# iagostorch/VVC-Affine-GPU

Hardware: AMD Instinct MI355X
Metric: candidate CU-blocks/s at 1080p QP32; bit-exact CPMV/cost match vs reference (higher is better)
Workload: dtype int32; 1 GPU; 1920x1080 QP32, 2 frames, 2-CPMV affine only (FULL+HALF CUs); resolution=1920x1080, qp=32, sequence_frames=2, sequence_pairs=3, pocs_rank0=2, modes=2cp, parallelism=frame-shard x1 (a sequence of its own per rank)

## Files before the change

### profiles/count_preds.py

```python
#!/usr/bin/env python3
import argparse
import ctypes
import json
import os
import sys

R = os.path.dirname(os.path.dirname(os.path.abspath(__file__)))
sys.path.insert(0, os.path.join(R, "vvc-affine-gpu_amd"))
sys.path.insert(0, R)

import torch

from bench import CONFIGS
from vame import _lib
from vame.engine import Engine
from vame.metrics import pair_accounting
from vame.seqrun import ShardRun


def main():
    ap = argparse.ArgumentParser()
    ap.add_argument("--config", default="c2", choices=sorted(CONFIGS))
    ap.add_argument("--qp", type=int, default=None)
    ap.add_argument("--gpus", type=int, default=1)
    ap.add_argument("--rank-only", type=int, default=0, help="count rank K's block of a --gpus N job")
    args = ap.parse_args()
    cfg = CONFIGS[args.config]
    qp = cfg["qp"] if args.qp is None else args.qp
    L = _lib.lib()
    if not hasattr(L, "vame_debug_pred_count"):
        raise SystemExit("VAME_LIB must point at the instrumentation build (make count)")
    L.vame_debug_pred_count.argtypes = [ctypes.c_void_p, ctypes.c_int]
    torch.cuda.set_device(0)
    dev = torch.device("cuda", 0)
    eng = Engine(cfg["W"], cfg["H"], 0)
    n_pairs = None
    if cfg["scaling"] == "weak":
        from vame.shard import frames_for_pairs, sequence_pairs
        n_pairs = sequence_pairs(cfg["frames"]) * args.gpus
    frames = cfg["frames"] if n_pairs is None else frames_for_pairs(n_pairs)
    run = ShardRun(eng, cfg["W"], cfg["H"], qp, frames, cfg["modes"], args.gpus, args.rank_only, dev,
                   n_pairs=n_pairs)
    cnt = (ctypes.c_ulonglong * 20)()
    L.vame_debug_pred_count(cnt, 1)
    run.step()
    torch.cuda.synchronize()
    L.vame_debug_pred_count(cnt, 1)
    acc = pair_accounting(cfg["W"], cfg["H"], (2, 3) if cfg["modes"] & 2 else (2,))
    alg_q, alg_b = acc["sb_pred_quad"] * run.pairs, acc["sb_pred_big"] * run.pairs
    out = {"config": args.config, "qp": qp, "pairs": run.pairs, "rank": [args.rank_only, args.gpus],
           "executed_quad": cnt[0], "algorithmic_quad": alg_q, "executed_pred_frac_quad": cnt[0] / alg_q,
           "executed_ctu": cnt[1], "algorithmic_ctu": alg_b, "executed_pred_frac_ctu": cnt[1] / alg_b,
           "executed_pred_frac": (cnt[0] + cnt[1]) / (alg_q + alg_b),
           "outside_tile_frac_quad": (cnt[2] + cnt[3]) / max(cnt[0], 1),
           "outside_tile_frac_ctu": (cnt[4] + cnt[5]) / max(cnt[1], 1),
           "outside_tile_quad_2cp_3cp": [cnt[2], cnt[3]], "outside_tile_ctu_2cp_3cp": [cnt[4], cnt[5]],
           "outside_held_by_wider_margin_quad": [cnt[6], cnt[7], cnt[8]],
           "outside_held_by_wider_margin_ctu": [cnt[9], cnt[10], cnt[11]],
           "lane_use_quad": cnt[0] / max(cnt[12], 1), "lane_use_ctu": cnt[1] / max(cnt[13], 1),
           "multi_cu_wave_slots_frac_quad": cnt[14] / max(cnt[12], 1),
           "multi_cu_wave_lane_use_quad": cnt[16] / max(cnt[14], 1)}
    print(json.dumps(out))
    eng.close()


if __name__ == "__main__":
    main()
```

### vvc-affine-gpu_amd/csrc/vame_engine.hip

```cpp
#include <hip/hip_ext.h>
#include <hip/hip_runtime.h>

#include <algorithm>
#include <cstdio>
#include <cstdlib>
#include <cstring>
#include <vector>

#include "../../include/vame.h"
#include "vame_kernel.h"
#include "vame_mc_core.h"
#include "vame_partition.h"
#include "vame_bipred.h"
#include "vame_ctx.h"
#include "vame_templates.h"

#if VAME_SPLIT_TU
namespace vame {
VAME_2CP_KERNELS(extern)
}
#endif

using namespace vame;

// ... 403 lines not shown
      pa.ref = jb.refs[r];
      pa.lambda = jb.lambda;
      for (int m = 0; m < 4; m++) {
        pa.cost[m] = jb.out->cost[r][m];
        pa.cpmv[m] = reinterpret_cast<vame_cpmvs_dev*>(jb.out->cpmvs[r][m]);
      }
      const bool last = j == njobs - 1 && r == jb.nrefs - 1;
      if (kp.nPairs == c->maxPairs || last) {
        kps.push_back(kp);
        kp.nPairs = 0;
      }
    }
  }
  return launch(c, kps, doFull, doHalf, doFull, (hipStream_t)stream);
}

int vame_affine_me_poc(vame_ctx* c, const uint16_t* cur, const uint16_t* const* refs, int nrefs,
                       float lambda, int mode_mask, int extra, const vame_poc_result* out,
                       void* stream) {
  if (!out) return VAME_E_INVALID;
  const vame_poc_job job{cur, refs, nrefs, lambda, out};
  return vame_affine_me_batch(c, &job, 1, mode_mask, extra, stream);
}

int vame_set_prof(vame_ctx* c, int enable) {
  if (!c) return VAME_E_INVALID;
  c->prof = enable != 0;
  return VAME_OK;
}

int vame_set_timing(vame_ctx* c, int enable) {
  if (!c) return VAME_E_INVALID;
  const bool keep = (enable & VAME_TIMING_KEEP) != 0;
  enable &= ~VAME_TIMING_KEEP;
  c->timing = enable == 2 ? (1 | 64) : enable != 0 ? (1 << kTimingClasses) - 1 : 0;
  if (!keep)
    for (size_t& u : c->evUsed) u = 0;
  return VAME_OK;
}

int vame_get_timing(vame_ctx* c, int cls, double* total_ms, int* launches, int reset) {
  if (!c || cls < 0 || cls >= kTimingClasses || !total_ms || !launches) return VAME_E_INVALID;
  DeviceGuard guard(c->device);
  VAME_HIP(guard.err);
  double t = 0;
  for (size_t i = 0; i < c->evUsed[cls]; i++) {
    float ms = 0;
    VAME_HIP(hipEventSynchronize(c->ev[cls][i].second));
    VAME_HIP(hipEventElapsedTime(&ms, c->ev[cls][i].first, c->ev[cls][i].second));
    t += ms;
  }
  *total_ms = t;
  *launches = (int)c->evUsed[cls];
  if (reset) c->evUsed[cls] = 0;
  return VAME_OK;
}

const char* vame_strerror(int code) {
  switch (code) {
    case VAME_OK: return "ok";
    case VAME_E_INVALID: return "invalid argument";
    case VAME_E_DEVICE: return "HIP runtime error";
    case VAME_E_NOMEM: return "out of memory";
    case VAME_E_UNSUPPORTED: return "unsupported";
    default: return "unknown error";
  }
}

const char* vame_last_hip_error(void) { return g_hip_err; }

#if VAME_PHASE_TIMING
int vame_debug_phase_cycles(unsigned long long* out, int reset) {
  if (!out) return VAME_E_INVALID;
  VAME_HIP(hipDeviceSynchronize());
  VAME_HIP(hipMemcpyFromSymbol(out, HIP_SYMBOL(g_phase_cycles), sizeof(g_phase_cycles)));
  if (reset) {
    unsigned long long z[7 * kPhSlots] = {};
    VAME_HIP(hipMemcpyToSymbol(HIP_SYMBOL(g_phase_cycles), z, sizeof(z)));
  }
  return VAME_OK;
}
#endif
#if VAME_COUNT_PRED
int vame_debug_pred_count(unsigned long long* out20, int reset) {
  if (!out20) return VAME_E_INVALID;
  VAME_HIP(hipDeviceSynchronize());
  VAME_HIP(hipMemcpyFromSymbol(out20, HIP_SYMBOL(g_pred_count), sizeof(unsigned long long) * 20));
  if (reset) {
    unsigned long long z[20] = {};
    VAME_HIP(hipMemcpyToSymbol(HIP_SYMBOL(g_pred_count), z, sizeof(z)));
  }
  return VAME_OK;
}
#endif
const char* vame_version(void) { return "vame 0.1 (gfx950)"; }

}
```

### vvc-affine-gpu_amd/csrc/vame_instr.h

```cpp
#pragma once
#include <hip/hip_runtime.h>

namespace vame {

#ifndef VAME_ABLATE
#define VAME_ABLATE 0
#endif
#ifndef VAME_DUP
#define VAME_DUP 0
#endif

#ifndef VAME_COUNT_PRED
#define VAME_COUNT_PRED 0
#endif
#if VAME_COUNT_PRED
__device__ unsigned long long g_pred_count[20];
#define PC_DECL unsigned pc_n = 0, pc_w = 0, pc_mw = 0, pc_me = 0;
#define PC_ADD                                                           \
  {                                                                      \
    pc_n++;                                                              \
    const unsigned long long m_ = __builtin_amdgcn_ballot_w64(true);     \
    if (__lane_id() == __builtin_ctzll(m_)) {                            \
      pc_w += 64;                                                        \
      if (!coop && logS < 6) {                                           \
        pc_mw += 64;                                                     \
        pc_me += __popcll(m_);                                           \
      }                                                                  \
    }                                                                    \
  }
#define PC_FLUSH                                                                                \
  {                                                                                             \
    if (pc_n) atomicAdd(&g_pred_count[REGION == 128], (unsigned long long)pc_n);               \
    if (pc_w) atomicAdd(&g_pred_count[12 + (REGION == 128)], (unsigned long long)pc_w);        \
    if (pc_mw) atomicAdd(&g_pred_count[14 + (REGION == 128)], (unsigned long long)pc_mw);      \
    if (pc_me) atomicAdd(&g_pred_count[16 + (REGION == 128)], (unsigned long long)pc_me);      \
  }
#else
#define PC_DECL
#define PC_ADD
#define PC_FLUSH
#endif

#ifndef VAME_PHASE_TIMING
#define VAME_PHASE_TIMING 0
#endif
enum { kPhStage, kPhPredict, kPhCost, kPhGradient, kPhSolve, kPhTail, kPhReduce, kNumPhases };
#if VAME_PHASE_TIMING
constexpr int kPhSlots = 2 * kNumPhases + 4;
__device__ unsigned long long g_phase_cycles[7][kPhSlots];
#define PH_DECL unsigned long long ph_acc[2 * kNumPhases] = {}; unsigned long long ph_t = __builtin_amdgcn_s_memtime(); const unsigned long long ph_t0 = ph_t;
#define PH_MARK(i) { const unsigned long long t_ = __builtin_amdgcn_s_memtime(); ph_acc[(i) + ph_off] += t_ - ph_t; ph_t = t_; }
__shared__ unsigned long long s_ph_blk[3];
__shared__ int s_ph_done;
#define PH_FLUSH { \
  if (lane == 0) { \
    for (int i_ = 0; i_ < 2 * kNumPhases; i_++) atomicAdd(&g_phase_cycles[KIND][i_], ph_acc[i_]); \
    const unsigned long long t1_ = __builtin_amdgcn_s_memtime(); \
    atomicMax(&s_ph_blk[1], t1_); \
    atomicAdd(&s_ph_blk[2], t1_ - ph_t0); \
    const int nw_ = (int)(blockDim.x >> 6); \
    if (atomicAdd(&s_ph_done, 1) == nw_ - 1) { \
      atomicAdd(&g_phase_cycles[KIND][2 * kNumPhases], (unsigned long long)nw_ * (s_ph_blk[1] - s_ph_blk[0])); \
      atomicAdd(&g_phase_cycles[KIND][2 * kNumPhases + 1], s_ph_blk[2]); \
      atomicAdd(&g_phase_cycles[KIND][2 * kNumPhases + 2], 1ull); \
      atomicAdd(&g_phase_cycles[KIND][2 * kNumPhases + 3], s_ph_blk[1] - s_ph_blk[0]); \
    } \
  } }
#define PH_INIT { if (tid == 0) { s_ph_blk[0] = ~0ull; s_ph_blk[1] = 0; s_ph_blk[2] = 0; s_ph_done = 0; } }
#define PH_START { if (lane == 0) atomicMin(&s_ph_blk[0], ph_t0); }
#elif defined(VAME_ISA_MARKS)
#define PH_DECL
#define PH_MARK(i) asm volatile("; PHASE_END " #i);
#define PH_FLUSH
#define PH_INIT
#define PH_START
#else
#define PH_DECL
#define PH_MARK(i)
#define PH_FLUSH
#define PH_INIT
#define PH_START
#endif

}
```

### vvc-affine-gpu_amd/csrc/vame_items.h

```cpp
#pragma once
#include <stdint.h>

namespace vame {

constexpr int kMaxCu = 16;
constexpr int kMaxTasks = 16;
constexpr int kTaskCu = 4;
constexpr int kItemCu = kMaxTasks * kTaskCu;
constexpr int kThreads = 256;

struct CuSlot {
  uint8_t x, y;
  uint8_t lw : 4, lh : 4;
  uint8_t align : 1;
  uint8_t taskCus : 5;
  uint16_t outOff : 9;
  uint16_t taskLogL : 4;
  uint16_t pad;
};
static_assert(sizeof(CuSlot) == 8, "CuSlot packing");

struct Item {
  int16_t nCu;
  int16_t rx, ry;
  int16_t coop;
  int16_t nTasks;
  int16_t rw, rh;
  int16_t pad;
  CuSlot cu[kItemCu];
};

enum { kKindQuad = 0, kKindCtu = 1, kKindHalf = 2, kKindCtu2 = 3, kKindHalf2W = 4, kKindHalf2H = 5, kKindQuad2 = 6 };
template <int KIND>
struct Cfg {
  static constexpr bool HALF2 = KIND == kKindHalf2W || KIND == kKindHalf2H;
  static constexpr bool QUAD = KIND == kKindQuad || KIND == kKindQuad2;
  static constexpr int REGION = QUAD ? 64 : 128;
  static constexpr int THREADS = QUAD || HALF2 ? 256 : KIND == kKindCtu ? 1024 : 512;
  static constexpr int SBL = KIND == kKindCtu2 || HALF2 || KIND == kKindQuad2 ? 2 : 1;
  static constexpr int MAXCU = (KIND == kKindHalf || KIND == kKindCtu2 || HALF2) ? 1 : kMaxCu;
  static constexpr int ITEMCU = QUAD ? kItemCu : MAXCU;
  static constexpr bool AUTO = QUAD;
  static constexpr bool COOP = KIND != kKindQuad2;
  static constexpr int MARGIN = 16;
  static constexpr int TILE = REGION + 2 * MARGIN;
  static constexpr int TILE_W = KIND == kKindHalf2H ? 64 + 2 * MARGIN : TILE;
  static constexpr int TILE_H = KIND == kKindHalf2W ? 64 + 2 * MARGIN : TILE;
  static constexpr int TP = (TILE_W + 7) / 16 * 16 + 8;
  static constexpr int TILE_ELEMS = TILE_H * TP + 16;
  static constexpr int NSB = THREADS * SBL;
  static constexpr bool STASH = KIND != kKindQuad2 && !HALF2;
};

struct BiCand {
  int32_t xy;
  int32_t shape;
  int32_t row;
  int32_t first;
};

}
```

### vvc-affine-gpu_amd/csrc/vame_kernel.h

```cpp
#pragma once
#include <hip/hip_runtime.h>

#include "vame_dev.h"
#include "vame_items.h"

namespace vame {

struct PairArgs {
  const uint16_t* cur;
  const uint16_t* ref;
  int64_t* cost[4];
  vame_cpmvs_dev* cpmv[4];
  float lambda;
  int32_t pad;
};
constexpr int kMaxPairs = 32;

struct KParams {
  PairArgs pair[kMaxPairs];
  const vame_cpmvs_dev* prev[2];
  int32_t* bestS;
  const Item* items;
  const int32_t* order;
  int nItems, nCtus, nPairs;
  int groupPairs, groupPer;
  int nChunks, cpp;
  int W, H, ctusPerRow;
  int extra;
  int run2, run3;
};

constexpr int kSolvePrio = 3;

struct CuState {
  int32_t cur[6];
  int32_t prev[6];
  int32_t best[6];
  int64_t bestCost;
  int64_t bestCostSnap;
  int32_t satd;
  int32_t inframe;
  int32_t live;
  int32_t rate;
  int32_t bestSatd;
  int32_t bestHasS;
  int32_t seedSkip;
  int32_t pad;
};

template <int LOGS>
__device__ __forceinline__ int seg_sum_c(int v) {
  if (LOGS > 0) v += dpp32<0x111, 0xF>(v);
  if (LOGS > 1) v += dpp32<0x112, 0xF>(v);
  if (LOGS > 2) v += dpp32<0x114, 0xF>(v);
  if (LOGS > 3) v += dpp32<0x118, 0xF>(v);
  if (LOGS > 4) v += dpp32<0x142, 0xA>(v);
  if (LOGS > 5) v += dpp32<0x143, 0xC>(v);
  return v;
}


constexpr unsigned long long kLaneBitMask[2] = {0xAAAAAAAAAAAAAAAAull, 0xCCCCCCCCCCCCCCCCull};
template <int B>
__device__ __forceinline__ int sel_bit(int if0, int if1) {
  int r;
  asm("v_cndmask_b32_e64 %0, %1, %2, %3" : "=v"(r) : "v"(if0), "v"(if1), "s"(kLaneBitMask[B]));
  return r;
}
template <int B>
__device__ __forceinline__ long long sel_bit64(long long if0, long long if1) {
  const int lo = sel_bit<B>((int)(unsigned long long)if0, (int)(unsigned long long)if1);
  const int hi = sel_bit<B>((int)((unsigned long long)if0 >> 32), (int)((unsigned long long)if1 >> 32));
  return (long long)(((unsigned long long)(unsigned)hi << 32) | (unsigned)lo);
}
template <int B>
__device__ __forceinline__ long long partner64(long long v) {
  static_assert(B == 0 || B == 1, "quad bits only");
  constexpr int ctrl = B == 1 ? 0x4E : 0xB1;
  const int lo = (int)(unsigned long long)v, hi = (int)((unsigned long long)v >> 32);
  const int rl = dpp32<ctrl, 0xF>(lo), rh = dpp32<ctrl, 0xF>(hi);
  return (long long)(((unsigned long long)(unsigned)rh << 32) | (unsigned)rl);
}
template <int B>
__device__ __forceinline__ long long xchg_masked64(long long a, long long b) {
  unsigned al = (unsigned)(unsigned long long)a, ah = (unsigned)((unsigned long long)a >> 32);
  const unsigned bl = (unsigned)(unsigned long long)b, bh = (unsigned)((unsigned long long)b >> 32);
  if constexpr (B == 3) {
// ... 257 lines not shown
  const int CPR = w.tileW / 8;
  const int NCH = w.tileH * CPR;
  if (w.regionOut) return;
#pragma unroll
  for (int j = 0; j < kStagePer<KIND>; j++) {
    const int ch = tid + j * C::THREADS;
    if (ch < NCH) *reinterpret_cast<uint4*>(&s_tile[(ch / CPR) * C::TP + (ch % CPR) * 8]) = tv[j];
  }
}

template <int KIND>
__device__ __forceinline__ void publish_item(const Item* it, int tid, CuSlot* s_cu, uint4* s_coef,
                                             uint8_t* s_eqmap, int* s_hdr, long long* s_val) {
  using C = Cfg<KIND>;
  if (tid < C::ITEMCU) s_cu[tid] = it->cu[tid];
  if (tid < 48) s_coef[tid] = reinterpret_cast<const uint4*>(&kCoefTab)[tid];
  if (tid < 76) s_eqmap[tid] = kEqMap.v[tid];
  if (tid == 0) {
    s_hdr[0] = it->coop | (it->nTasks << 16);
    s_hdr[1] = 4;
  }
  for (int i = tid; i < C::MAXCU * kNumMom; i += C::THREADS) s_val[i] = 0;
}

struct TaskCtx {
  int tid, lane, wv;
  int cuB, cuE;
  int logL;
  int logS;
  int nCuW;
  int myCu;
  int local;
  int sbIdx;
  int sx, sy;
  int sbCols;
  bool active;
  bool leader;
  Geo g;
};
template <int KIND>
__device__ __forceinline__ TaskCtx task_lanes(const ItemCtx& w, int tid, bool coop, const CuSlot* s_cu) {
  constexpr int SBL = Cfg<KIND>::SBL;
  TaskCtx t;
  t.tid = tid;
  t.lane = tid & 63;
  t.wv = tid >> 6;
  const int lidx = coop ? tid : t.lane;
  const CuSlot t0 = s_cu[coop ? 0 : t.wv * kTaskCu];
  int cuB = coop ? 0 : t.wv * kTaskCu;
  int cuE = cuB + t0.taskCus;
  int logL = t0.taskLogL;
  t.cuB = __builtin_amdgcn_readfirstlane(cuB);
  t.cuE = __builtin_amdgcn_readfirstlane(cuE);
  t.logL = __builtin_amdgcn_readfirstlane(logL);
  t.logS = min(t.logL, 6);
  t.nCuW = coop ? (t.wv == 0 ? t.cuE : 0) : t.cuE - t.cuB;
  const int kLane = t.cuB + (lidx >> t.logL);
  t.myCu = kLane < t.cuE ? kLane : -1;
  t.g.x = t.g.y = t.g.lw = t.g.lh = t.g.w = t.g.h = 0;
  t.local = lidx & ((1 << t.logL) - 1);
  t.sbIdx = 0;
  t.sx = 0;
  t.sy = 0;
  t.sbCols = 1;
  t.active = false;
  if (t.myCu >= 0) {
    const CuSlot cs = s_cu[t.myCu];
    t.g.lw = cs.lw;
    t.g.lh = cs.lh;
    t.g.w = 1 << t.g.lw;
    t.g.h = 1 << t.g.lh;
    t.g.x = w.ctuX + cs.x;
    t.g.y = w.ctuY + cs.y;
    t.sbIdx = tid;
    t.sbCols = 1 << (t.g.lw - 2);
    t.sx = (t.local & (t.sbCols - 1)) << 2;
    t.sy = (t.local >> (t.g.lw - 2)) << (SBL == 2 ? 3 : 2);
    t.active = (t.g.x + t.g.w <= w.W) && (t.g.y + t.g.h <= w.H);
  }
  t.leader = t.myCu >= 0 && (t.lane & ((1 << t.logS) - 1)) == (1 << t.logS) - 1;
  return t;
}

template <int KIND>
__device__ __forceinline__ void take_task_slots(int next, int li, int dstBase, CuSlot* s_cu) {
  if (li < kTaskCu) s_cu[dstBase + li] = s_cu[min(next, Cfg<KIND>::ITEMCU / kTaskCu - 1) * kTaskCu + li];
}

__device__ __forceinline__ int seg_sum(int logS, int v) {
  return logS == 4 ? seg_sum_c<4>(v) : logS == 5 ? seg_sum_c<5>(v) : seg_sum_c<6>(v);
}
__device__ __forceinline__ uint4 ext_row_dpp(const uint2& p) {
  return ext_row(p, dpp32<0x138, 0xF>((int)p.y), dpp32<0x130, 0xF>((int)p.x));
}
__device__ __forceinline__ int bcast_lane7(int v) { return __builtin_amdgcn_update_dpp(0, v, 0x157, 0xF, 0xF, false); }

template <int SBL>
__device__ __forceinline__ void publish_rows(const uint2 (&Pr)[SBL][4], int idx, uint2* s_top, uint2* s_bot,
                                             uint4 (&X)[6]) {
  if constexpr (SBL == 1) {
#pragma unroll
    for (int r = 0; r < 4; r++) X[r + 1] = ext_row_dpp(Pr[0][r]);
  }
  s_top[idx] = Pr[0][0];
  s_bot[idx] = Pr[SBL - 1][3];
}

template <int THREADS>
__device__ __forceinline__ void edge_rows(int idx, int sbCols, const uint2* s_top, const uint2* s_bot, uint2& tb,
                                          uint2& bt) {
  tb = s_bot[max(idx - sbCols, 0)];
  bt = s_top[min(idx + sbCols, THREADS - 1)];
}

template <int ncp, bool STORE>
__device__ __forceinline__ int update_lanes(int loc, const double* M, CuState& st, int cx, int cy, int W, int H) {
  int f = 0, q = 0;
  if (loc < 2 * ncp) {
    const int j = loc;
    const double d = M[j == 1 ? 2 : j == 2 ? 1 : j];
    const int cj = st.cur[j], pj = st.prev[j];
    const int v = update_cpmv(cj, d, (j & 1) ? cy : cx, (j & 1) ? H : W);
    f = (v != cj ? 1 : 0) | (v != pj ? 16 : 0);
    if constexpr (STORE) {
      st.prev[j] = cj;
      st.cur[j] = v;
    }
    q = to_quarter(v);
  }
  const int q2 = dpp32<0x112, 0xF>(q), q4 = dpp32<0x114, 0xF>(q);
  if (loc < 2 * ncp) f += eg_bits(q - (loc >= 4 ? q4 : loc >= 2 ? q2 : 0)) << 8;
  f += dpp32<0x111, 0xF>(f);
  f += dpp32<0x112, 0xF>(f);
  f += dpp32<0x114, 0xF>(f);
  return f;
}

template <int ncp, bool coop, bool keepS, int kDup>
__device__ __forceinline__ bool solve_update_phase(const ItemCtx& w, const TaskCtx& t, const CuSlot* s_cu,
                                                   CuState* s_st, long long (*s_val)[kNumMom], double (*s_mat)[42],
                                                   const uint8_t* s_eqmap) {
  int cuS = t.myCu, loc = t.local;
  opaque(cuS);
  opaque(loc);
  const bool solver = cuS >= 0 && loc < 64;
  const bool act = solver && s_st[cuS].live;
  const int Ls = 1 << t.logS;
  double dd[6] = {0, 0, 0, 0, 0, 0};
  long long* V = s_val[cuS < 0 ? 0 : cuS];
  double* M = s_mat[cuS < 0 ? 0 : cuS];
  const CuSlot cs = s_cu[cuS < 0 ? 0 : cuS];
  if constexpr ((kDup & 16) != 0) {
    double dd2[6] = {0, 0, 0, 0, 0, 0};
    double* M2 = M;
    seg_solve<ncp, true>(V, M2, s_eqmap, loc, Ls, act, coop, cs.lw, cs.lh, dd2);
    asm volatile("" ::"v"(dd2[0]), "v"(dd2[1]), "v"(dd2[3]));
    wave_sync();
  }
  seg_solve<ncp>(V, M, s_eqmap, loc, Ls, act, coop, cs.lw, cs.lh, dd);
  if (keepS && coop && solver && loc == 7) {
    CuState& st = s_st[cuS];
    st.bestCostSnap = st.bestCost;
    st.satd = 0;
  }
  const int cx = w.ctuX + cs.x, cy = w.ctuY + cs.y;
  if constexpr ((kDup & 2048) != 0) {
// ... 34 lines not shown
  const CuSlot cs = s_cu[k];
  const int mode = cs.align * 2 + (ncp - 2);
  const size_t idx = (size_t)w.ctu * (cs.align ? kHalfCusPerCtu : kFullCusPerCtu) + cs.outOff;
  pa.cost[mode][idx] = st.bestCost;
  vame_cpmvs_dev o;
  o.ncps = ncp;
  o.ltx = st.best[0]; o.lty = st.best[1]; o.rtx = st.best[2];
  o.rty = st.best[3]; o.lbx = st.best[4]; o.lby = st.best[5];
  pa.cpmv[mode][idx] = o;
}

template <int KIND, bool PROF, int MODE, typename L>
__device__ __forceinline__ void affine_me_body(const KParams& p, L& lds) {
  constexpr bool run2 = (MODE & 1) != 0, run3 = (MODE & 2) != 0;
  using C = Cfg<KIND>;
  constexpr int REGION = C::REGION;
  (void)REGION;
  static_assert((C::TP * 2) % 16 == 0 && C::TILE_W % 8 == 0, "16-byte tile rows");
  constexpr int SBL = C::SBL;
  constexpr bool STASH = SBL == 2 && C::STASH;
  using Own = Lds<KIND, run2 && run3>;
  static_assert(sizeof(L::tile) >= sizeof(Own::tile) && sizeof(L::top) >= sizeof(Own::top) &&
                    sizeof(L::bestS) >= sizeof(Own::bestS) && sizeof(L::pred) >= sizeof(Own::pred) &&
                    sizeof(L::val) >= sizeof(Own::val) && sizeof(L::mat) >= sizeof(Own::mat) &&
                    sizeof(L::st) >= sizeof(Own::st) && sizeof(L::cu) >= sizeof(Own::cu),
                "LDS layout too small for this kernel class");
  uint16_t* s_tile = lds.tile;
  uint2* s_top = lds.top;
  uint2* s_bot = lds.bot;
  auto& s_bestS = lds.bestS;
  auto& s_pred = lds.pred;
  auto& s_val = lds.val;
  auto& s_mat = lds.mat;
  uint4* s_coef = lds.coef;
  uint8_t* s_eqmap = lds.eqmap;
  CuState* s_st = lds.st;
  CuSlot* s_cu = lds.cu;
  int* s_hdr = lds.hdr;
  __shared__ long long s_dup[(VAME_DUP & 4) ? kNumMom : 1];

  const int tid = threadIdx.x;
  [[maybe_unused]] const int lane = tid & 63;
  const int wv = tid >> 6;
  constexpr int ph_off = 0;
  (void)ph_off;
  PH_DECL
  PC_DECL

  ItemCtx w;
  if (!locate_item<KIND>(p, w)) return;
  const PairArgs& pa = p.pair[w.pairIdx];
  const uint16_t* __restrict__ ref = w.ref;
  const uint16_t* __restrict__ cur = w.cur;
  const int W = w.W, H = w.H, ctu = w.ctu, ctuX = w.ctuX, ctuY = w.ctuY, pairIdx = w.pairIdx, itemIdx = w.itemIdx;
  const int tx0 = w.tx0, ty0 = w.ty0, tileW = w.tileW, tileH = w.tileH;
  uint4 tv[kStagePer<KIND>];
  if constexpr ((VAME_DUP & 64) != 0) {
    int tid2 = tid;
    opaque(tid2);
    stage_load<KIND>(w, tid2, tv);
    stage_store<KIND>(w, tid2, tv, s_tile);
    __syncthreads();
  }
  stage_load<KIND>(w, tid, tv);
  publish_item<KIND>(w.it, tid, s_cu, s_coef, s_eqmap, s_hdr, &s_val[0][0]);
  PH_INIT
  stage_store<KIND>(w, tid, tv, s_tile);
  __syncthreads();
  PH_START
  const int hdr = __builtin_amdgcn_readfirstlane(s_hdr[0]);
  const int nTasks = (hdr >> 16) & 0xFF;
  const bool coop = C::COOP && (!C::AUTO || (hdr & 1) != 0);
  const bool claim = C::AUTO && (hdr & 2) != 0;
  PH_MARK(kPhStage)
  if (!coop && wv >= nTasks) {
    PH_FLUSH
    return;
  }

  const int tidItem = tid;
  for (int task = coop ? 0 : __builtin_amdgcn_readfirstlane(wv);;) {
    int tidTask = tidItem;
    opaque(tidTask);
    const TaskCtx t = task_lanes<KIND>(w, tidTask, coop, s_cu);
    const int tid = t.tid, lane = t.lane, wv = t.wv, cuB = t.cuB, logS = t.logS, nCuW = t.nCuW;
    const int myCu = t.myCu, local = t.local, sbIdx = t.sbIdx, sx = t.sx, sy = t.sy, sbCols = t.sbCols;
    const bool active = t.active, leader = t.leader;
    const Geo g = t.g;
    auto run_pass = [&](auto ncpTag, auto coopTag, auto keepTag) {
      constexpr int ncp = decltype(ncpTag)::value;
      constexpr bool coop = decltype(coopTag)::value;
      constexpr bool keepS = decltype(keepTag)::value;
      constexpr int ph_off = ncp == 3 ? kNumPhases : 0;
      (void)ph_off;
      constexpr int kDup = (VAME_DUP & 32) && ncp != 3 ? 0 : VAME_DUP;
      const int niter = (ncp == 3 ? 4 : 5) + p.extra;

      if (lane < nCuW) {
        int k = __lane_id();
        opaque(k);
        k += cuB;
        const CuSlot cs = s_cu[k];
        CuState& st = s_st[k];
        const int cx = ctuX + cs.x, cy = ctuY + cs.y;
        int c[6] = {0, 0, 0, 0, 0, 0};
        if (ncp == 3) {
          int prev[4];
          if (run2) {
            for (int i = 0; i < 4; i++) prev[i] = st.best[i];
          } else {
            const vame_cpmvs_dev& pv =
                p.prev[cs.align][(size_t)ctu * (cs.align ? kHalfCusPerCtu : kFullCusPerCtu) + cs.outOff];
            prev[0] = pv.ltx; prev[1] = pv.lty; prev[2] = pv.rtx; prev[3] = pv.rty;
          }
          int lbx, lby;
          derive_lb(prev[0], prev[1], prev[2], prev[3], cs.lw, cs.lh, cx, cy, W, H, lbx, lby);
          c[0] = prev[0]; c[1] = prev[1]; c[2] = prev[2]; c[3] = prev[3]; c[4] = lbx; c[5] = lby;
          int skip = 0, satd0 = 0;
          if (run2 && st.bestHasS) {
            const int hx = shl(prev[2] - prev[0], 7 - cs.lw), hy = shl(prev[3] - prev[1], 7 - cs.lw);
            const int vx = shl(lbx - prev[0], 7 - cs.lh), vy = shl(lby - prev[1], 7 - cs.lh);
            if (vx == -hy && vy == hx) {
              skip = 1;
              satd0 = st.bestSatd;
            }
          }
          st.seedSkip = skip;
          st.satd = satd0;
        } else {
          st.satd = 0;
          st.bestHasS = 0;
        }
        int never = (int)0x80000000;
        int costInit = (int)kCostInit;
        opaque(never);
        opaque(costInit);
        for (int i = 0; i < 6; i++) {
          st.cur[i] = c[i];
          st.prev[i] = never;
          st.best[i] = c[i];
        }
        st.bestCost = (long long)costInit;
        st.bestCostSnap = (long long)costInit;
        st.rate = affine_bits(c, ncp);
        st.inframe = (cx + (1 << cs.lw) <= W) && (cy + (1 << cs.lh) <= H);
        st.live = st.inframe;
      }
      phase_sync(coop);

      for (int iter = 0; iter <= niter; iter++) {
        uint2 Pr[SBL][4], Og[SBL][4];
        uint4 X[6];
        const bool live = active && s_st[myCu < 0 ? 0 : myCu].live;
        const bool reuse = ncp == 3 && iter == 0 && s_st[myCu < 0 ? 0 : myCu].seedSkip;
        if (live && !reuse && !(VAME_ABLATE & 8)) {
          PC_ADD
          Geo gp = g;
          int sxp = sx, syp = sy;
          opaque_geo(gp, sxp, syp);
          int cp[6];
          for (int i = 0; i < 6; i++) cp[i] = s_st[myCu].cur[i];
          const MvField f = mv_field(cp, ncp, gp.lw, gp.lh);
          if constexpr ((kDup & 128) != 0) {
            int cp2[6];
            for (int i = 0; i < 6; i++) cp2[i] = cp[i];
            int lw2 = gp.lw;
            opaque(cp2[0]);
            opaque(lw2);
            const MvField f2 = mv_field(cp2, ncp, lw2, gp.lh);
            if (ncp == 3)
              asm volatile("" ::"v"(f2.bx), "v"(f2.by), "v"(f2.hx), "v"(f2.hy), "v"(f2.vx), "v"(f2.vy),
                           "v"((int)f2.spread));
            else
              asm volatile("" ::"v"(f2.bx), "v"(f2.by), "v"(f2.hx), "v"(f2.hy), "v"((int)f2.spread));
          }
          int satdLane = 0;
#pragma unroll
          for (int j = 0; j < SBL; j++) {
            bool outside;
            satdLane += predict_sb<C::TILE, C::TP, PROF, (VAME_ABLATE & 1024) != 0 && ncp == 3, ncp>(
                f, sxp, syp + 4 * j, gp, s_tile, tx0, ty0, tileW - 9, tileH - 9, ref, cur, W, H, s_coef, Pr[j],
                Og[j], outside);
            if (SBL == 2 && j == 0) {
#pragma unroll
              for (int r = 0; r < 4; r++)
                if constexpr (STASH) s_pred[r][sbIdx] = Pr[0][r];
            }
#if VAME_COUNT_PRED
            {
              const unsigned long long out = __builtin_amdgcn_ballot_w64(outside);
              if (out && __lane_id() == __builtin_ctzll(__builtin_amdgcn_ballot_w64(true)))
                atomicAdd(&g_pred_count[2 + 2 * (REGION == 128) + (ncp == 3)], (unsigned long long)__popcll(out));
            }
            if (j > 0) PC_ADD
#endif
          }
          if (kDup & 1) {
            MvField f2 = f;
            opaque(f2.bx);
            uint2 P2[4], O2[4];
            bool out2;
            int s2 = predict_sb<C::TILE, C::TP, PROF>(f2, sxp, syp, gp, s_tile, tx0, ty0, tileW - 9, tileH - 9,
                                                      ref, cur, W, H, s_coef, P2, O2, out2);
            s2 += (int)(P2[0].x ^ P2[3].y ^ O2[1].x);
            asm volatile("" ::"v"(s2));
          }
          publish_rows<SBL>(Pr, sbIdx, s_top, s_bot, X);
          if constexpr ((kDup & 256) != 0) {
            int i2 = sbIdx;
            opaque(i2);
            uint2 Q[SBL][4];
#pragma unroll
            for (int j = 0; j < SBL; j++)
#pragma unroll
              for (int r = 0; r < 4; r++) {
                Q[j][r] = Pr[j][r];
                opaque(reinterpret_cast<int&>(Q[j][r].x));
              }
            uint4 X2[6];
            publish_rows<SBL>(Q, i2, s_top, s_bot, X2);
            if constexpr (SBL == 1) {
#pragma unroll
              for (int r = 0; r < 4; r++) asm volatile("" ::"v"(X2[r + 1].x), "v"(X2[r + 1].w));
            }
          }
          if constexpr ((kDup & 512) != 0) {
            int s2 = satdLane;
            opaque(s2);
            const int v2 = seg_sum(logS, s2);
            asm volatile("" ::"v"(v2));
          }
          const int v = seg_sum(logS, satdLane);
          if (leader) {
            if (coop)
              atomicAdd(&s_st[myCu].satd, v);
            else
              s_st[myCu].satd = v;
          }
        }
        phase_sync(coop);
        PH_MARK(kPhPredict)

        const bool lastIter = iter == niter;
        bool better = false;
        if constexpr ((kDup & 1024) != 0) {
          int bet2 = 0;
          if (myCu >= 0 && (keepS || local == 7)) {
            const CuState& st = s_st[myCu];
            int r2 = st.rate;
            opaque(r2);
            if (iter == 0 || st.live) bet2 = price(st.satd, pa.lambda, r2) < st.bestCost;
          }
          if (!keepS) bet2 = bcast_lane7(bet2);
          asm volatile("" ::"v"(bet2));
        }
        if constexpr (!keepS) {
          int bet = 0;
          if (myCu >= 0 && local == 7) {
            CuState& st = s_st[myCu];
            if (iter == 0 || st.live) {
              const long long cost = price(st.satd, pa.lambda, st.rate);
              if (cost < st.bestCost) {
                st.bestCost = cost;
                bet = 1;
              }
            }
            st.satd = 0;
          }
          bet = bcast_lane7(bet);
          if (myCu >= 0 && local < 6 && bet) s_st[myCu].best[local] = s_st[myCu].cur[local];
        } else {
          if (myCu >= 0) {
            CuState& st = s_st[myCu];
            if (iter == 0 || st.live) {
              const long long cost = price(st.satd, pa.lambda, st.rate);
              better = cost < (coop ? st.bestCostSnap : st.bestCost);
              if (better && local == 7) {
                st.bestCost = cost;
                st.bestSatd = st.satd;
                st.bestHasS = !lastIter && st.live;
              }
            }
            if (local < 6 && better) st.best[local] = st.cur[local];
          }
        }
        PH_MARK(kPhCost)
        if (lastIter) {
          phase_sync(coop);
          break;
        }

        {
          int S[SBL][5];
#pragma unroll
          for (int j = 0; j < SBL; j++)
#pragma unroll
            for (int k = 0; k < 5; k++) S[j][k] = 0;
          char* gBest = SBL == 2 ? reinterpret_cast<char*>(p.bestS + ((size_t)(pairIdx * p.nCtus + ctu) * p.nItems +
                                                                      itemIdx) * 5 * C::NSB)
                                 : nullptr;
          auto gbest = [&](int k, int j) -> int32_t& {
            int i = sbIdx;
            opaque(i);
            return *reinterpret_cast<int32_t*>(gBest + (unsigned)(k * C::NSB + j * C::THREADS + i) * 4u);
          };
          if (reuse && live) {
#pragma unroll
            for (int j = 0; j < SBL; j++)
#pragma unroll
              for (int k = 0; k < 5; k++) S[j][k] = SBL == 1 ? s_bestS[k][sbIdx] : gbest(k, j);
          } else if (live && !(VAME_ABLATE & 2)) {
            int nbIdx = sbIdx;
            if constexpr (SBL == 2) opaque(nbIdx);
            uint2 tb, bt;
            edge_rows<C::THREADS>(nbIdx, sbCols, s_top, s_bot, tb, bt);
            X[0] = ext_row_dpp(tb);
            if constexpr ((kDup & 256) != 0) {
              int n2 = nbIdx;
              opaque(n2);
              uint2 tb2, bt2;
              edge_rows<C::THREADS>(n2, sbCols, s_top, s_bot, tb2, bt2);
              const uint4 a2 = ext_row_dpp(tb2), b2 = ext_row_dpp(bt2);
              asm volatile("" ::"v"(a2.x), "v"(a2.w), "v"(b2.x), "v"(b2.w));
            }
            Geo gg = g;
            int sxg = sx, syg = sy;
            if constexpr (SBL == 2) opaque_geo(gg, sxg, syg);
            if constexpr (SBL == 1) {
              X[5] = ext_row_dpp(bt);
              grad_sb(sxg, syg, gg, X, Og[0], S[0]);
            } else {
#pragma unroll
              for (int j = 0; j < SBL; j++) {
                if (STASH && j == 0) {
#pragma unroll
                  for (int r = 0; r < 4; r++) Pr[0][r] = s_pred[r][sbIdx];
                }
#pragma unroll
                for (int r = 0; r < 4; r++)
                  X[r + 1] = ext_row_dpp(Pr[j][r]);
                X[5] = ext_row_dpp(j + 1 < SBL ? Pr[j + 1][0] : bt);
                {
                  const unsigned b0 = (unsigned)((gg.y + syg + 4 * j) * W + gg.x + sxg) * 2u, bw = (unsigned)W * 2u;
                  const char* base = reinterpret_cast<const char*>(cur);
#pragma unroll
                  for (int r = 0; r < 4; r++) Og[j][r] = *reinterpret_cast<const uint2*>(base + (b0 + (unsigned)r * bw));
                }
                grad_sb(sxg, syg + 4 * j, gg, X, Og[j], S[j]);
                if (j + 1 < SBL) X[0] = X[4];
              }
            }
            if (kDup & 2) {
              int S2[5];
              int sxd = sxg;
              opaque(sxd);
              grad_sb(sxd, syg, gg, X, Og[0], S2);
              asm volatile("" ::"v"(S2[0] ^ S2[1] ^ S2[2] ^ S2[3] ^ S2[4]));
            }
            if (keepS && better && !(SBL == 2 && (VAME_ABLATE & 2048))) {
#pragma unroll
              for (int j = 0; j < SBL; j++)
#pragma unroll
                for (int k = 0; k < 5; k++) {
                  if constexpr (SBL == 1)
                    s_bestS[k][sbIdx] = S[j][k];
                  else
                    gbest(k, j) = S[j][k];
                }
            }
          }
          PH_MARK(kPhGradient)
          if (!(VAME_ABLATE & 4)) {
            long long* dst = s_val[myCu < 0 ? 0 : myCu];
            int va[SBL];
#pragma unroll
            for (int j = 0; j < SBL; j++) va[j] = sy + 2 + 4 * j;
            if (ncp == 2)
              reduce_equations<2, SBL>(S, sx + 2, va, logS, myCu >= 0, coop, dst);
            else
              reduce_equations<3, SBL>(S, sx + 2, va, logS, myCu >= 0, coop, dst);
            if constexpr ((kDup & 4) != 0) {
              int ud = sx + 2;
              opaque(ud);
              if (ncp == 2)
                reduce_equations<2, SBL>(S, ud, va, logS, myCu >= 0, coop, s_dup);
              else
                reduce_equations<3, SBL>(S, ud, va, logS, myCu >= 0, coop, s_dup);
            }
          }
        }
        phase_sync(coop);
        PH_MARK(kPhReduce)

        __builtin_amdgcn_s_setprio(kSolvePrio);
        if (!(VAME_ABLATE & 1)) {
          const bool liveNew = solve_update_phase<ncp, coop, keepS, kDup>(w, t, s_cu, s_st, s_val, s_mat, s_eqmap);
          if (!coop) {
            if (__ballot(liveNew) == 0) {
              __builtin_amdgcn_s_setprio(0);
              break;
            }
          }
        }
        __builtin_amdgcn_s_setprio(0);
        phase_sync(coop);
        PH_MARK(kPhSolve)
        if (coop && !any_cu_live(t, s_st)) break;
      }
      write_results<ncp>(pa, w, t, s_cu, s_st);
      phase_sync(coop);
      PH_MARK(kPhTail)
    };
    using I2 = std::integral_constant<int, 2>;
    using I3 = std::integral_constant<int, 3>;
    using T = std::true_type;
    using F = std::false_type;
    using KeepS = std::integral_constant<bool, run3>;
    if (C::COOP && coop) {
      if constexpr (C::COOP) {
        if constexpr (run2) run_pass(I2{}, T{}, KeepS{});
        if constexpr (run3) run_pass(I3{}, T{}, F{});
      }
    } else {
      if constexpr (run2) run_pass(I2{}, F{}, KeepS{});
      if constexpr (run3) run_pass(I3{}, F{}, F{});
    }
    if (!C::QUAD) break;
    int next = task + (coop ? 1 : 4);
    if (claim) {
      int v = 0;
      if (lane == 0) v = atomicAdd(&s_hdr[1], 1);
      next = __builtin_amdgcn_readfirstlane(v);
    }
    if (next >= nTasks) break;
    if (coop) {
      take_task_slots<KIND>(next, tid, 0, s_cu);
      __syncthreads();
    } else {
      take_task_slots<KIND>(next, lane, wv * kTaskCu, s_cu);
      wave_sync();
    }
    task = next;
  }
  PH_FLUSH
  PC_FLUSH
}

__device__ __forceinline__ bool quad_item_sbl2(const KParams& p) {
  const int b = blockIdx.x;
  const int gr = b % (p.nItems * p.groupPer);
  return (p.items[gr / p.groupPer].coop & 4) != 0;
}
template <int MODE>
constexpr bool kQuadMerged = MODE == 1;
template <int MODE>
__global__ __launch_bounds__(kThreads) __attribute__((amdgpu_waves_per_eu(4))) void affine_me_quad(
    KParams p) {
  __shared__ Lds<kKindQuad, MODE == 3> lds;
  if constexpr (kQuadMerged<MODE>) {
    if (quad_item_sbl2(p)) {
      affine_me_body<kKindQuad2, false, MODE>(p, lds);
      return;
    }
  }
  affine_me_body<kKindQuad, false, MODE>(p, lds);
}
template <int MODE>
__global__ __launch_bounds__(kThreads) __attribute__((amdgpu_waves_per_eu(4))) void affine_me_quad2(
    KParams p) {
  __shared__ Lds<kKindQuad2, MODE == 3> lds;
  affine_me_body<kKindQuad2, false, MODE>(p, lds);
}
template <int MODE>
__global__ __launch_bounds__(512) __attribute__((amdgpu_waves_per_eu(4))) void affine_me_ctu2(KParams p) {
  __shared__ Lds<kKindCtu2, MODE == 3> lds;
  affine_me_body<kKindCtu2, false, MODE>(p, lds);
}
template <int MODE>
__global__ __launch_bounds__(256) __attribute__((amdgpu_waves_per_eu(4))) void affine_me_half2w(KParams p) {
  __shared__ Lds<kKindHalf2W, MODE == 3> lds;
  affine_me_body<kKindHalf2W, false, MODE>(p, lds);
}
template <int MODE>
__global__ __launch_bounds__(256) __attribute__((amdgpu_waves_per_eu(4))) void affine_me_half2h(KParams p) {
  __shared__ Lds<kKindHalf2H, MODE == 3> lds;
  affine_me_body<kKindHalf2H, false, MODE>(p, lds);
}
template <int MODE>
__global__ __launch_bounds__(256) __attribute__((amdgpu_waves_per_eu(4))) void affine_me_half2(KParams p) {
  __shared__ Lds<kKindHalf2H, MODE == 3> lds;
  const int gr = blockIdx.x % (p.nItems * p.groupPer);
  const Item& it = p.items[gr / p.groupPer];
  if (it.rw > it.rh)
    affine_me_body<kKindHalf2W, false, MODE>(p, lds);
  else
    affine_me_body<kKindHalf2H, false, MODE>(p, lds);
}
template <int MODE>
__global__ __launch_bounds__(kThreads) __attribute__((amdgpu_waves_per_eu(4))) void affine_me_quad_prof(
    KParams p) {
  __shared__ Lds<kKindQuad, MODE == 3> lds;
  affine_me_body<kKindQuad, true, MODE>(p, lds);
}
template <int MODE>
__global__ __launch_bounds__(1024) void affine_me_ctu_prof(KParams p) {
  __shared__ Lds<kKindCtu, MODE == 3> lds;
  affine_me_body<kKindCtu, true, MODE>(p, lds);
}
template <int MODE>
__global__ __launch_bounds__(512) __attribute__((amdgpu_waves_per_eu(4))) void affine_me_half_prof(KParams p) {
  __shared__ Lds<kKindHalf, MODE == 3> lds;
  affine_me_body<kKindHalf, true, MODE>(p, lds);
}

#if VAME_COUNT_PRED || VAME_PHASE_TIMING
#define VAME_SPLIT_TU 0
#else
#define VAME_SPLIT_TU 1
#endif
#define VAME_2CP_KERNELS(X)                 \
// ... 6 lines not shown
```

Baseline: 231.5 million CU-blocks/s.

## Relayout quad SBL2 waves to one subblock per lane once few CUs remain live

For the 2-CPMV quad kernel in non-cooperative waves, after each solve step the code checks whether the surviving CUs fit in 64 lanes at one subblock per lane. If they do, it remaps lanes to CUs and subblocks, and switches predict, gradient, publish and reduce to a single-subblock path for the rest of the iterations. This is meant to halve per-lane serial work in late iterations when most CUs have converged, at the cost of extra branching, register pressure and remap logic. It also adds instrumentation counters for SBL2 lane use.

```diff
diff --git a/profiles/count_preds.py b/profiles/count_preds.py
--- a/profiles/count_preds.py
+++ b/profiles/count_preds.py
@@ -41,7 +41,7 @@
     frames = cfg["frames"] if n_pairs is None else frames_for_pairs(n_pairs)
     run = ShardRun(eng, cfg["W"], cfg["H"], qp, frames, cfg["modes"], args.gpus, args.rank_only, dev,
                    n_pairs=n_pairs)
-    cnt = (ctypes.c_ulonglong * 20)()
+    cnt = (ctypes.c_ulonglong * 24)()
     L.vame_debug_pred_count(cnt, 1)
     run.step()
     torch.cuda.synchronize()
@@ -59,7 +59,12 @@
            "outside_held_by_wider_margin_ctu": [cnt[9], cnt[10], cnt[11]],
            "lane_use_quad": cnt[0] / max(cnt[12], 1), "lane_use_ctu": cnt[1] / max(cnt[13], 1),
            "multi_cu_wave_slots_frac_quad": cnt[14] / max(cnt[12], 1),
-           "multi_cu_wave_lane_use_quad": cnt[16] / max(cnt[14], 1)}
+           "multi_cu_wave_lane_use_quad": cnt[16] / max(cnt[14], 1),
+           "sbl2_wave_iters_quad": cnt[18], "sbl2_wave_iters_le64_quad": cnt[19],
+           "sbl2_wave_iters_le64_iter0_quad": cnt[20],
+           "sbl2_wave_lane_use_quad": cnt[22] / max(cnt[21], 1),
+           "sbl2_wave_iters_relaid_quad": cnt[23],
+           "sbl1_multi_cu_wave_lane_use_quad": (cnt[16] - cnt[22]) / max(cnt[14] - cnt[21], 1)}
     print(json.dumps(out))
     eng.close()
 
diff --git a/vvc-affine-gpu_amd/csrc/vame_engine.hip b/vvc-affine-gpu_amd/csrc/vame_engine.hip
--- a/vvc-affine-gpu_amd/csrc/vame_engine.hip
+++ b/vvc-affine-gpu_amd/csrc/vame_engine.hip
@@ -509,12 +509,12 @@
 }
 #endif
 #if VAME_COUNT_PRED
-int vame_debug_pred_count(unsigned long long* out20, int reset) {
-  if (!out20) return VAME_E_INVALID;
+int vame_debug_pred_count(unsigned long long* out24, int reset) {
+  if (!out24) return VAME_E_INVALID;
   VAME_HIP(hipDeviceSynchronize());
-  VAME_HIP(hipMemcpyFromSymbol(out20, HIP_SYMBOL(g_pred_count), sizeof(unsigned long long) * 20));
+  VAME_HIP(hipMemcpyFromSymbol(out24, HIP_SYMBOL(g_pred_count), sizeof(unsigned long long) * 24));
   if (reset) {
-    unsigned long long z[20] = {};
+    unsigned long long z[24] = {};
     VAME_HIP(hipMemcpyToSymbol(HIP_SYMBOL(g_pred_count), z, sizeof(z)));
   }
   return VAME_OK;
diff --git a/vvc-affine-gpu_amd/csrc/vame_instr.h b/vvc-affine-gpu_amd/csrc/vame_instr.h
--- a/vvc-affine-gpu_amd/csrc/vame_instr.h
+++ b/vvc-affine-gpu_amd/csrc/vame_instr.h
@@ -14,19 +14,31 @@
 #define VAME_COUNT_PRED 0
 #endif
 #if VAME_COUNT_PRED
-__device__ unsigned long long g_pred_count[20];
-#define PC_DECL unsigned pc_n = 0, pc_w = 0, pc_mw = 0, pc_me = 0;
+__device__ unsigned long long g_pred_count[24];
+#define PC_DECL unsigned pc_n = 0, pc_w = 0, pc_mw = 0, pc_me = 0, pc2[6] = {};
 #define PC_ADD                                                           \
   {                                                                      \
     pc_n++;                                                              \
     const unsigned long long m_ = __builtin_amdgcn_ballot_w64(true);     \
     if (__lane_id() == __builtin_ctzll(m_)) {                            \
       pc_w += 64;                                                        \
-      if (!coop && logS < 6) {                                           \
+      if (!coop && pcLogS < 6) {                                         \
         pc_mw += 64;                                                     \
         pc_me += __popcll(m_);                                           \
       }                                                                  \
     }                                                                    \
+  }
+#define PC2_ITER(m_, per_, iter_)                                                        \
+  {                                                                                      \
+    const unsigned long long l_ = (m_);                                                  \
+    if (l_ && __lane_id() == __builtin_ctzll(l_)) {                                      \
+      const unsigned sb_ = (unsigned)__popcll(l_) * (per_);         \
+      pc2[0]++;                                                                          \
+      if (sb_ <= 64u) pc2[(iter_) == 0 ? 2 : 1]++;                                       \
+      pc2[3] += 64u * (per_);                                                            \
+      pc2[4] += sb_;                                                                     \
+      if ((per_) == 1) pc2[5]++;                                                         \
+    }                                                                                    \
   }
 #define PC_FLUSH                                                                                \
   {                                                                                             \
@@ -34,10 +46,13 @@
     if (pc_w) atomicAdd(&g_pred_count[12 + (REGION == 128)], (unsigned long long)pc_w);        \
     if (pc_mw) atomicAdd(&g_pred_count[14 + (REGION == 128)], (unsigned long long)pc_mw);      \
     if (pc_me) atomicAdd(&g_pred_count[16 + (REGION == 128)], (unsigned long long)pc_me);      \
+    for (int i_ = 0; i_ < 6; i_++)                                                              \
+      if (pc2[i_]) atomicAdd(&g_pred_count[18 + i_], (unsigned long long)pc2[i_]);              \
   }
 #else
 #define PC_DECL
 #define PC_ADD
+#define PC2_ITER(m_, per_, iter_)
 #define PC_FLUSH
 #endif
 
diff --git a/vvc-affine-gpu_amd/csrc/vame_items.h b/vvc-affine-gpu_amd/csrc/vame_items.h
--- a/vvc-affine-gpu_amd/csrc/vame_items.h
+++ b/vvc-affine-gpu_amd/csrc/vame_items.h
@@ -52,6 +52,18 @@
   static constexpr bool STASH = KIND != kKindQuad2 && !HALF2;
 };
 
+constexpr bool relayout_fits(unsigned liveCus, int logNsb) {
+  return liveCus != 0 && (__builtin_popcount(liveCus) << logNsb) <= 64;
+}
+struct RelayoutLane {
+  int cu;
+  int sb;
+};
+constexpr RelayoutLane relayout_lane(int lane, unsigned liveCus, int logNsb) {
+  const unsigned m = (lane >> logNsb) ? liveCus & (liveCus - 1) : liveCus;
+  return {m ? __builtin_ctz(m) : -1, lane & ((1 << logNsb) - 1)};
+}
+
 struct BiCand {
   int32_t xy;
   int32_t shape;
diff --git a/vvc-affine-gpu_amd/csrc/vame_kernel.h b/vvc-affine-gpu_amd/csrc/vame_kernel.h
--- a/vvc-affine-gpu_amd/csrc/vame_kernel.h
+++ b/vvc-affine-gpu_amd/csrc/vame_kernel.h
@@ -3,6 +3,10 @@
 
 #include "vame_dev.h"
 #include "vame_items.h"
+
+#ifndef VAME_RELAYOUT
+#define VAME_RELAYOUT 1
+#endif
 
 namespace vame {
 
@@ -426,6 +430,33 @@
   return t;
 }
 
+__device__ __forceinline__ void relayout_task(const ItemCtx& w, unsigned liveCus, const CuSlot* s_cu, TaskCtx& t) {
+  const int logNsb = t.logL + 1;
+  const RelayoutLane rl = relayout_lane((int)__lane_id(), liveCus, logNsb);
+  t.logL = t.logS = logNsb;
+  t.myCu = rl.cu < 0 ? -1 : t.cuB + rl.cu;
+  t.local = rl.sb;
+  t.sbIdx = t.myCu >= 0 ? t.tid : 0;
+  t.g.x = t.g.y = t.g.lw = t.g.lh = t.g.w = t.g.h = 0;
+  t.sx = 0;
+  t.sy = 0;
+  t.sbCols = 1;
+  t.active = t.myCu >= 0;
+  if (t.myCu >= 0) {
+    const CuSlot cs = s_cu[t.myCu];
+    t.g.lw = cs.lw;
+    t.g.lh = cs.lh;
+    t.g.w = 1 << t.g.lw;
+    t.g.h = 1 << t.g.lh;
+    t.g.x = w.ctuX + cs.x;
+    t.g.y = w.ctuY + cs.y;
+    t.sbCols = 1 << (t.g.lw - 2);
+    t.sx = (t.local & (t.sbCols - 1)) << 2;
+    t.sy = (t.local >> (t.g.lw - 2)) << 2;
+  }
+  t.leader = t.myCu >= 0 && (t.lane & ((1 << logNsb) - 1)) == (1 << logNsb) - 1;
+}
+
 template <int KIND>
 __device__ __forceinline__ void take_task_slots(int next, int li, int dstBase, CuSlot* s_cu) {
   if (li < kTaskCu) s_cu[dstBase + li] = s_cu[min(next, Cfg<KIND>::ITEMCU / kTaskCu - 1) * kTaskCu + li];
@@ -626,11 +657,12 @@
   for (int task = coop ? 0 : __builtin_amdgcn_readfirstlane(wv);;) {
     int tidTask = tidItem;
     opaque(tidTask);
-    const TaskCtx t = task_lanes<KIND>(w, tidTask, coop, s_cu);
-    const int tid = t.tid, lane = t.lane, wv = t.wv, cuB = t.cuB, logS = t.logS, nCuW = t.nCuW;
-    const int myCu = t.myCu, local = t.local, sbIdx = t.sbIdx, sx = t.sx, sy = t.sy, sbCols = t.sbCols;
-    const bool active = t.active, leader = t.leader;
-    const Geo g = t.g;
+    TaskCtx t = task_lanes<KIND>(w, tidTask, coop, s_cu);
+    const int tid = t.tid, lane = t.lane, wv = t.wv, cuB = t.cuB, nCuW = t.nCuW;
+    int sbIdx = t.sbIdx, logS = t.logS, myCu = t.myCu, local = t.local, sx = t.sx, sy = t.sy, sbCols = t.sbCols;
+    bool active = t.active, leader = t.leader;
+    Geo g = t.g;
+    [[maybe_unused]] const int pcLogS = t.logS;
     auto run_pass = [&](auto ncpTag, auto coopTag, auto keepTag) {
       constexpr int ncp = decltype(ncpTag)::value;
       constexpr bool coop = decltype(coopTag)::value;
@@ -639,6 +671,8 @@
       (void)ph_off;
       constexpr int kDup = (VAME_DUP & 32) && ncp != 3 ? 0 : VAME_DUP;
       const int niter = (ncp == 3 ? 4 : 5) + p.extra;
+      constexpr bool kRelay = VAME_RELAYOUT && KIND == kKindQuad2 && MODE == 1 && ncp == 2 && !coop;
+      [[maybe_unused]] bool relaid = false;
 
       if (lane < nCuW) {
         int k = __lane_id();
@@ -697,6 +731,11 @@
         uint4 X[6];
         const bool live = active && s_st[myCu < 0 ? 0 : myCu].live;
         const bool reuse = ncp == 3 && iter == 0 && s_st[myCu < 0 ? 0 : myCu].seedSkip;
+#if VAME_COUNT_PRED
+        if constexpr (KIND == kKindQuad2 && ncp == 2) {
+          if (!coop && pcLogS < 6) PC2_ITER(__builtin_amdgcn_ballot_w64(live), relaid ? 1u : 2u, iter)
+        }
+#endif
         if (live && !reuse && !(VAME_ABLATE & 8)) {
           PC_ADD
           Geo gp = g;
@@ -721,6 +760,7 @@
           int satdLane = 0;
 #pragma unroll
           for (int j = 0; j < SBL; j++) {
+            if (kRelay && j > 0 && relaid) break;
             bool outside;
             satdLane += predict_sb<C::TILE, C::TP, PROF, (VAME_ABLATE & 1024) != 0 && ncp == 3, ncp>(
                 f, sxp, syp + 4 * j, gp, s_tile, tx0, ty0, tileW - 9, tileH - 9, ref, cur, W, H, s_coef, Pr[j],
@@ -749,7 +789,12 @@
             s2 += (int)(P2[0].x ^ P2[3].y ^ O2[1].x);
             asm volatile("" ::"v"(s2));
           }
-          publish_rows<SBL>(Pr, sbIdx, s_top, s_bot, X);
+          if (kRelay && relaid) {
+            s_top[sbIdx] = Pr[0][0];
+            s_bot[sbIdx] = Pr[0][3];
+          } else {
+            publish_rows<SBL>(Pr, sbIdx, s_top, s_bot, X);
+          }
           if constexpr ((kDup & 256) != 0) {
             int i2 = sbIdx;
             opaque(i2);
@@ -883,7 +928,8 @@
 #pragma unroll
                 for (int r = 0; r < 4; r++)
                   X[r + 1] = ext_row_dpp(Pr[j][r]);
-                X[5] = ext_row_dpp(j + 1 < SBL ? Pr[j + 1][0] : bt);
+                const bool below = j + 1 < SBL && !(kRelay && relaid);
+                X[5] = ext_row_dpp(below ? Pr[j + 1 < SBL ? j + 1 : j][0] : bt);
                 {
                   const unsigned b0 = (unsigned)((gg.y + syg + 4 * j) * W + gg.x + sxg) * 2u, bw = (unsigned)W * 2u;
                   const char* base = reinterpret_cast<const char*>(cur);
@@ -891,6 +937,7 @@
                   for (int r = 0; r < 4; r++) Og[j][r] = *reinterpret_cast<const uint2*>(base + (b0 + (unsigned)r * bw));
                 }
                 grad_sb(sxg, syg + 4 * j, gg, X, Og[j], S[j]);
+                if (kRelay && relaid) break;
                 if (j + 1 < SBL) X[0] = X[4];
               }
             }
@@ -919,7 +966,12 @@
             int va[SBL];
 #pragma unroll
             for (int j = 0; j < SBL; j++) va[j] = sy + 2 + 4 * j;
-            if (ncp == 2)
+            if (kRelay && relaid) {
+              int S1[1][5], v1[1] = {va[0]};
+#pragma unroll
+              for (int k = 0; k < 5; k++) S1[0][k] = S[0][k];
+              reduce_equations<2, 1>(S1, sx + 2, v1, logS, myCu >= 0, coop, dst);
+            } else if (ncp == 2)
               reduce_equations<2, SBL>(S, sx + 2, va, logS, myCu >= 0, coop, dst);
             else
               reduce_equations<3, SBL>(S, sx + 2, va, logS, myCu >= 0, coop, dst);
@@ -940,9 +992,21 @@
         if (!(VAME_ABLATE & 1)) {
           const bool liveNew = solve_update_phase<ncp, coop, keepS, kDup>(w, t, s_cu, s_st, s_val, s_mat, s_eqmap);
           if (!coop) {
-            if (__ballot(liveNew) == 0) {
+            const unsigned long long liveBal = __ballot(liveNew);
+            if (liveBal == 0) {
               __builtin_amdgcn_s_setprio(0);
               break;
+            }
+            if constexpr (kRelay) {
+              if (!relaid && t.logL < 6 && (__popcll(liveBal) << (t.logL + 1)) <= 64) {
+                unsigned liveCus = 0;
+                for (int k = 0; k < (64 >> t.logL); k++)
+                  liveCus |= (unsigned)((liveBal >> ((k << t.logL) + 7)) & 1) << k;
+                relayout_task(w, liveCus, s_cu, t);
+                sbIdx = t.sbIdx; logS = t.logS; myCu = t.myCu; local = t.local; sx = t.sx; sy = t.sy; sbCols = t.sbCols;
+                active = t.active; leader = t.leader; g = t.g;
+                relaid = true;
+              }
             }
           }
         }
@@ -980,6 +1044,11 @@
     if (coop) {
       take_task_slots<KIND>(next, tid, 0, s_cu);
       __syncthreads();
+    } else if constexpr (VAME_RELAYOUT && KIND == kKindQuad2 && MODE == 1) {
+      int tidEnd = tidItem;
+      opaque(tidEnd);
+      take_task_slots<KIND>(next, tidEnd & 63, (tidEnd >> 6) * kTaskCu, s_cu);
+      wave_sync();
     } else {
       take_task_slots<KIND>(next, lane, wv * kTaskCu, s_cu);
       wave_sync();
```

Result: faster. 237.3 million CU-blocks/s (median of 6 runs) (+2.5%).
